# dwofk/fast-depth

Measured on NVIDIA H100. Metric: depth-maps/sec @224x224 b64, higher is better.
Workload: dtype f16

## Files before the change

### fastdepth_b200/_lib.py

```python
import ctypes
import os

HERE = os.path.dirname(os.path.abspath(__file__))
LIB_PATH = os.environ.get('FD_B200_LIB') or os.path.join(HERE, 'libfastdepth_b200.so')

FD_F32, FD_F16, FD_BF16 = 0, 1, 2
FD_STAGE_STEM, FD_STAGE_DWPW, FD_STAGE_HEAD, FD_STAGE_CONV, FD_STAGE_DECONV, FD_STAGE_UPCONV = 0, 1, 2, 3, 4, 5
FD_ACT_RELU, FD_ACT_RELU6 = 0, 1


class StageDesc(ctypes.Structure):
    _fields_ = [(n, ctypes.c_int32) for n in
                ('kind', 'c_in', 'c_out', 'ksize', 'stride', 'act', 'upsample', 'skip_src', 'skip_mode')]


_c_int_p = ctypes.POINTER(ctypes.c_int)
_c_float_p = ctypes.POINTER(ctypes.c_float)
_c_double_p = ctypes.POINTER(ctypes.c_double)
_vp = ctypes.c_void_p

SIGNATURES = {
    'fd_abi_version': (ctypes.c_int, []),
    'fd_last_error': (ctypes.c_char_p, []),
    'fd_plan_create': (ctypes.c_int, [ctypes.POINTER(StageDesc), ctypes.c_int, ctypes.c_int, ctypes.c_int,
                                      ctypes.c_int, ctypes.c_int, ctypes.c_int, ctypes.POINTER(_vp)]),
    'fd_plan_set_stage_weights': (ctypes.c_int, [_vp, ctypes.c_int, _vp, _vp, _vp, _vp, _vp, _vp]),
    'fd_plan_set_option': (ctypes.c_int, [_vp, ctypes.c_char_p, ctypes.c_int]),
    'fd_plan_get_option': (ctypes.c_int, [_vp, ctypes.c_char_p, _c_int_p]),
    'fd_forward': (ctypes.c_int, [_vp, _vp, _vp, _vp]),
    'fd_forward_batch': (ctypes.c_int, [_vp, ctypes.c_int, _vp, _vp, _vp]),
    'fd_forward_shape': (ctypes.c_int, [_vp, ctypes.c_int, ctypes.c_int, ctypes.c_int, _vp, _vp, _vp]),
    'fd_forward_host': (ctypes.c_int, [_vp, _vp, _vp, _vp]),
    'fd_pipeline_submit': (ctypes.c_int, [_vp, _vp, _vp, ctypes.POINTER(ctypes.c_uint64)]),
    'fd_pipeline_wait': (ctypes.c_int, [_vp, ctypes.c_uint64]),
    'fd_stage_buffer': (ctypes.c_int, [_vp, ctypes.c_int, ctypes.c_int, ctypes.POINTER(_vp),
                                       _c_int_p, _c_int_p, _c_int_p, _c_int_p, _c_int_p]),
    'fd_plan_launches_per_forward': (ctypes.c_int, [_vp, _c_int_p]),
    'fd_plan_workspace_bytes': (ctypes.c_int, [_vp, ctypes.POINTER(ctypes.c_size_t)]),
    'fd_plan_step_count': (ctypes.c_int, [_vp, _c_int_p]),
    'fd_plan_step_info': (ctypes.c_int, [_vp, ctypes.c_int, _c_int_p, _c_double_p, _c_double_p,
                                         ctypes.c_char_p, ctypes.c_int]),
    'fd_plan_step_macs': (ctypes.c_int, [_vp, ctypes.c_int, _c_double_p, _c_double_p]),
    'fd_plan_time_steps': (ctypes.c_int, [_vp, _vp, _vp, _vp, ctypes.c_int, ctypes.c_int, ctypes.c_int, _c_float_p]),
    'fd_plan_trace_stage': (ctypes.c_int, [_vp, ctypes.c_int, _vp, _vp, ctypes.POINTER(ctypes.c_uint64), ctypes.c_int,
                                           _c_int_p, _c_int_p]),
    'fd_debug_block_plan': (ctypes.c_int, [ctypes.c_int] * 8 + [_c_int_p, ctypes.c_int]),
    'fd_debug_conv_plan': (ctypes.c_int, [ctypes.c_int] * 7 + [_c_int_p, ctypes.c_int]),
    'fd_debug_convt_plan': (ctypes.c_int, [ctypes.c_int] * 8 + [_c_int_p, ctypes.c_int]),
    'fd_debug_pw_tf32x3_plan': (ctypes.c_int, [ctypes.c_int] * 7 + [_c_int_p, ctypes.c_int]),
    'fd_debug_pw_plan': (ctypes.c_int, [ctypes.c_int] * 7 + [_c_int_p, ctypes.c_int]),
    'fd_debug_conv_tf32x3_plan': (ctypes.c_int, [ctypes.c_int] * 9 + [_c_int_p, ctypes.c_int]),
    'fd_metrics_accumulate': (ctypes.c_int, [_vp, _vp, ctypes.c_int, ctypes.c_int, ctypes.c_int, _vp,
                                             ctypes.c_int, _vp]),
    'fd_nyu_val_gather': (ctypes.c_int, [_vp, _vp, _vp, _vp] + [ctypes.c_int] * 6 + [_vp, _vp, ctypes.c_int, _vp]),
    'fd_plan_destroy': (None, [_vp]),
}

_lib = None


def load():
    global _lib
    if _lib is not None:
        return _lib
    if not os.path.exists(LIB_PATH):
        raise RuntimeError(
            "fastdepth_b200: %s not found. Build it with `python -m fastdepth_b200.build` "
            "(or __graft_entry__.build()); there is no fallback path." % LIB_PATH)
    lib = ctypes.CDLL(LIB_PATH)
    for name, (res, args) in SIGNATURES.items():
# ... 14 lines not shown
```

### fastdepth_b200/build.py

```python
import os
import subprocess
import sys

HERE = os.path.dirname(os.path.abspath(__file__))
CSRC = os.path.join(HERE, 'csrc')
LIB = os.path.join(HERE, 'libfastdepth_b200.so')
SOURCES = ('fd_api.cu', 'fd_kernels_simt.cu', 'fd_block_tc.cu', 'fd_chain_tc.cu', 'fd_stem_tc.cu', 'fd_conv_tc.cu',
           'fd_metrics.cu')
NVCC_FLAGS = ['-gencode', 'arch=compute_90a,code=sm_90a', '-O3', '-lineinfo', '-std=c++17',
              '-Xcompiler', '-fPIC']


def _nvcc():
    for cand in (os.environ.get('NVCC'), '/usr/local/cuda/bin/nvcc', 'nvcc'):
        if cand and (os.path.isabs(cand) and os.path.exists(cand) or not os.path.isabs(cand)):
            return cand
    raise RuntimeError('nvcc not found')


def _stale(target, deps):
    if not os.path.exists(target):
        return True
    t = os.path.getmtime(target)
    return any(os.path.getmtime(d) > t for d in deps)


def build(force=False, verbose=False):
    srcs = [os.path.join(CSRC, s) for s in SOURCES]
    deps = srcs + [os.path.join(CSRC, f) for f in os.listdir(CSRC) if f.endswith(('.cuh', '.h'))]
    deps.append(os.path.join(os.path.dirname(HERE), 'include', 'fastdepth_b200.h'))
# ... 43 lines not shown
```

### fastdepth_b200/csrc/fd_api.cu

```cuda
#include <algorithm>
#include <cstring>
#include <functional>
#include <string>
#include <vector>

#include "fd_block_plan.h"
#include "fd_conv_plan.h"
#include "fd_common.cuh"

namespace fd {

BlockPlanOut block_tc_debug_plan(int ksize, int stride, int h_out, int w_out, int n, int c_in, int c_out, int head);
ConvPlanOut conv_tc_debug_plan(int kind, int ksize, int h_out, int w_out, int n, int c_in, int c_out, int n_sms);
ConvPlanOut pw_tf32x3_debug_plan(int h_out, int w_out, int n, int c_in, int c_out, int upsample, int n_sms);
ConvPlanOut pw_tc_debug_plan(int h_out, int w_out, int n, int c_in, int c_out, int upsample, int n_sms);
ConvPlanOut conv_tc_tf32x3_debug_plan(int kind, int ksize, int h_out, int w_out, int n, int c_in, int c_out, int upsample,
                                      int n_sms);

static thread_local std::string g_last_error;
void set_error(const std::string& msg) { g_last_error = msg; }
int fail(int code, const std::string& msg) {
    g_last_error = msg;
    return code;
}
// ... 13 lines not shown
                          int w_in, int oh, int ow, void* x, float* t, cudaStream_t st);
struct BlockTcPlan;
bool block_tc_supported(int dtype, const StageGeom& g, bool head_fused);
int block_tc_prepare(int dtype, const BlockArgs& a, const float* head_w, float head_scale, float head_bias, int head_act,
                     void* head_out, bool tma_epilogue, const TcLaunchOpts& opts, BlockTcPlan** out);
int block_tc_launch(BlockTcPlan* p, cudaStream_t st, void* head_out);
void block_tc_destroy(BlockTcPlan* p);
const char* block_tc_name(BlockTcPlan* p);
int block_tc_trace(BlockTcPlan* bp, cudaStream_t st, void* head_out, unsigned long long* out_host, int* rows, int* cols);
struct ChainTcPlan;
bool chain_tc_supported(int dtype, const StageGeom* g, int n_layers);
int chain_tc_prepare(int dtype, const BlockArgs* layers, int n_layers, const TcLaunchOpts& opts, ChainTcPlan** out);
int chain_tc_launch(ChainTcPlan* cp, cudaStream_t st);
void chain_tc_destroy(ChainTcPlan* cp);
const char* chain_tc_name(ChainTcPlan* cp);
int chain_tc_trace(ChainTcPlan* cp, cudaStream_t st, unsigned long long* out_host, int* rows, int* cols);
struct StemTcPlan;
bool stem_tc_supported(int dtype, const StageGeom& g);
int stem_tc_prepare(int dtype, const StageGeom& g, const float* w27_dev, const float* scale_dev, const float* bias_dev, void* out,
                    const TcLaunchOpts& opts, StemTcPlan** res);
int stem_tc_launch(StemTcPlan* sp, const void* x, cudaStream_t st);
void stem_tc_destroy(StemTcPlan* sp);
const char* stem_tc_name(StemTcPlan* sp);
struct ConvTcPlan;
bool conv_tc_supported(int dtype, const StageGeom& g, int kind);
int conv_tc_prepare(int dtype, int kind, const StageGeom& g, const void* in, const void* w, const float* scale_dev,
                    const float* bias_dev, void* out, const TcLaunchOpts& opts, ConvTcPlan** res);
int conv_tc_launch(ConvTcPlan* cp, cudaStream_t st);
void conv_tc_destroy(ConvTcPlan* cp);
const char* conv_tc_name(ConvTcPlan* cp);
bool pw_tf32x3_supported(const StageGeom& g);
bool conv_tc_tf32x3_supported(const StageGeom& g, int kind);
int conv_tc_tf32x3_prepare(int kind, const StageGeom& g, const void* in, const float* w_split, const float* scale_dev,
                           const float* bias_dev, void* out, const TcLaunchOpts& opts, ConvTcPlan** res);
int pw_tf32x3_prepare(const StageGeom& g, const void* mid, const float* w_split, const float* scale_dev, const float* bias_dev,
                      void* out, int out_pitch, int reduce, const TcLaunchOpts& opts, ConvTcPlan** res);
int tf32_split_weights(const float* w, size_t count, float* dst);
bool pw_tc_supported(int dtype, const StageGeom& g);
int pw_tc_prepare(int dtype, const StageGeom& g, const void* mid, const void* w, const float* scale_dev, const float* bias_dev,
                  void* out, int out_pitch, int reduce, const TcLaunchOpts& opts, ConvTcPlan** res);
int dw_mid_launch(int dtype, const BlockArgs& a, cudaStream_t st);
BlockPlanOut block_tc_plan_for(const StageGeom& g, const TcLaunchOpts& opts, bool* pinned);
size_t block_tc_param_bytes(BlockTcPlan* bp);
size_t chain_tc_param_bytes(ChainTcPlan* cp);
size_t stem_tc_param_bytes(StemTcPlan* sp);
size_t conv_tc_param_bytes(ConvTcPlan* cp);
// ... 9 lines not shown
    void* out = nullptr;
    void* out_alloc = nullptr;
    int out_c = 0;
    int out_pitch = 0;
    int concat_src = -1;
    void* mid = nullptr;
    float* dw_w = nullptr;
    float* dw_scale = nullptr;
    float* dw_bias = nullptr;
    void* pw_w = nullptr;
    float* pw_w_f32 = nullptr;
    float* pw_scale = nullptr;
    float* pw_bias = nullptr;
    float* w_split = nullptr;
    float head_scale = 0.f, head_bias = 0.f;
    bool have_weights = false;
};

struct StageRun {
    BlockTcPlan* tc = nullptr;
    StemTcPlan* stc = nullptr;
    ConvTcPlan* ctc = nullptr;
    ChainTcPlan* chain = nullptr;
    int chained = 0;
    void* out_eff = nullptr;
};

struct Step {
    int stage;
    std::string name;
    double alg_bytes, macs;
    double dw_macs = 0.0;
    std::function<int(cudaStream_t, const void*, void*)> run;
};

struct StageShape {
    StageGeom g{};
    int out_h = 0, out_w = 0;
    int out_c = 0;
};

struct StepSet {
    int n = 0, h = 0, w = 0;
    std::vector<Step> steps;
    std::vector<StageRun> runs;
    size_t bytes = 0;
    unsigned long long stamp = 0;
};

}

using namespace fd;

struct fd_plan {
    int n = 0, h = 0, w = 0, dtype = 0, device = 0, n_sms = 132;
    std::vector<Stage> stages;
    std::vector<StepSet*> sets;
    unsigned long long set_clock = 0;
    int opt_path = 1, opt_fold_head = 1, opt_graph = 1, opt_tma_epilogue = 1, opt_inplace_skip = 1, opt_pdl = 0, opt_wait_sleep_ns = 0;
    int opt_chain = 1;
    int opt_cluster = 1;
    int opt_tf32x3 = 0;
    int opt_unfuse = 1;
    size_t workspace_bytes = 0;
    size_t split_bytes = 0;
    struct PipeSlot { void* x = nullptr; void* y = nullptr; cudaEvent_t up = nullptr, done = nullptr, down = nullptr; bool busy = false; };
    PipeSlot pipe[3];
    cudaStream_t pipe_h2d = nullptr, pipe_run = nullptr, pipe_d2h = nullptr;
    unsigned long long pipe_next = 0;
    void* stage_x = nullptr;
    void* stage_y = nullptr;
    cudaEvent_t last_done = nullptr;
    cudaStream_t last_stream = nullptr;
    bool last_stream_set = false;
    void* l2_flush = nullptr;
    size_t l2_flush_bytes = 0;
    struct GraphEntry { const void* x; void* y; int n, h, w; cudaGraphExec_t exec; unsigned long long stamp; };
    std::vector<GraphEntry> graphs;
    unsigned long long graph_clock = 0;
    int graph_misses = 0;
};
static const size_t kMaxGraphs = 8;
static const size_t kUnfuseMaxMidBytes = size_t(16) << 20;
static const size_t kMaxStepSets = 8;

namespace fd {
// ... 5 lines not shown
        if (cudaGetDevice(&prev) != cudaSuccess) { ok = false; return; }
        if (prev != dev && cudaSetDevice(dev) != cudaSuccess) ok = false;
    }
    ~DeviceGuard() {
        if (prev >= 0) cudaSetDevice(prev);
    }
};

static int dev_alloc(fd_plan* p, void** ptr, size_t bytes) {
    bytes = (bytes + 255) & ~size_t(255);
    FD_CUDA_OK(cudaMalloc(ptr, bytes));
    FD_CUDA_OK(cudaMemset(*ptr, 0, bytes));
    FD_CUDA_OK(cudaStreamSynchronize(cudaStreamLegacy));
    p->workspace_bytes += bytes;
    return FD_OK;
}

static void destroy_set(StepSet* ss) {
    for (auto& r : ss->runs) {
        if (r.tc) block_tc_destroy(r.tc);
        if (r.stc) stem_tc_destroy(r.stc);
        if (r.ctc) conv_tc_destroy(r.ctc);
        if (r.chain) chain_tc_destroy(r.chain);
    }
    delete ss;
}

static StepSet* find_set(fd_plan* p, int n, int h, int w) {
    for (StepSet* ss : p->sets)
        if (ss->n == n && ss->h == h && ss->w == w) return ss;
    return nullptr;
}

static bool is_capacity_set(const fd_plan* p, const StepSet* ss) { return ss->n == p->n && ss->h == p->h && ss->w == p->w; }

static void invalidate(fd_plan* p) {
    for (auto& g : p->graphs) cudaGraphExecDestroy(g.exec);
    p->graphs.clear();
    for (StepSet* ss : p->sets) destroy_set(ss);
    p->sets.clear();
    for (auto& s : p->stages) { cudaFree(s.w_split); s.w_split = nullptr; }
    p->split_bytes = 0;
}

static int split_weights(fd_plan* p, Stage& s, size_t count, const float** out) {
    if (!s.w_split) {
// ... 67 lines not shown
            s.g.h_out = hh; s.g.w_out = ww;
        }
        s.out_h = s.g.h_out * (s.g.upsample || is_phased(d.kind) ? 2 : 1);
        s.out_w = s.g.w_out * (s.g.upsample || is_phased(d.kind) ? 2 : 1);
        s.out_c = d.c_out;
        if (d.skip_src >= 0) {
            if (d.kind != FD_STAGE_DWPW || !d.upsample || d.skip_src >= i) return fail(FD_ERR_INVALID, "bad skip_src");
            const StageShape& src = out[d.skip_src];
            if (src.out_h != s.out_h || src.out_w != s.out_w || (!d.skip_mode && src.g.c_out != d.c_out))
                return fail(FD_ERR_INVALID, "stage " + std::to_string(i) + ": skip tensor shape does not match the upsampled output");
            if (d.skip_mode) {
                if (d.skip_mode != 1 || concat_src[d.skip_src] >= 0 || stages[d.skip_src].skip_src >= 0)
                    return fail(FD_ERR_INVALID, "bad skip_mode / skip source");
                s.out_c = d.c_out + src.g.c_out;
                concat_src[d.skip_src] = i;
            }
        }
        ch = s.out_c; hh = s.out_h; ww = s.out_w;
    }
    if (hh != h || ww != w) return fail(FD_ERR_INVALID, "stage list does not return to the input resolution");
    return FD_OK;
}

static int build_steps(fd_plan* p, int n, int h, int w, StepSet* ss) {
    const int ns = (int)p->stages.size();
    const double es = (double)dtype_size(p->dtype);
    for (auto& s : p->stages)
        if (!s.have_weights) return fail(FD_ERR_STATE, "fd_plan_set_stage_weights was not called for every stage");
    ss->n = n; ss->h = h; ss->w = w;
    ss->runs.assign(ns, StageRun());
    std::vector<StageRun>& R = ss->runs;
    std::vector<fd_stage_desc> D(ns);
    for (int i = 0; i < ns; ++i) D[i] = p->stages[i].d;
    std::vector<StageShape> S;
    int wrc = walk_stages(D.data(), ns, n, h, w, S);
    if (wrc != FD_OK) return wrc;
    std::vector<StageGeom> G(ns);
    for (int i = 0; i < ns; ++i) G[i] = S[i].g;

    TcLaunchOpts lopts;
    lopts.pdl = p->opt_pdl; lopts.sleep_ns = p->opt_wait_sleep_ns; lopts.n_sms = p->n_sms; lopts.cluster = p->opt_cluster;
    Stage& head = p->stages[ns - 1];
    Stage& last = p->stages[ns - 2];
    const bool fold = p->opt_fold_head && (last.d.kind == FD_STAGE_DWPW || last.d.kind == FD_STAGE_CONV) && last.d.upsample &&
                      last.d.skip_src < 0;
    bool head_fused = false;

    for (int i = 0; i < ns; ++i) {
        Stage& s = p->stages[i];
        StageRun& r = R[i];
        StageGeom& sg = G[i];
        const void* in = i > 0 ? R[i - 1].out_eff : nullptr;
        r.out_eff = s.out;
        sg.in_pitch = i > 0 ? p->stages[i - 1].out_pitch : 0;
        sg.out_pitch = s.out_pitch;
        sg.skip_pitch = (s.d.skip_src >= 0 && !s.d.skip_mode) ? p->stages[s.d.skip_src].out_pitch : s.out_pitch;
        if (s.d.kind == FD_STAGE_STEM) {
            Step st;
            st.stage = i;
            st.name = "stem_kernel";
            st.macs = (double)sg.n * sg.h_out * sg.w_out * sg.c_out * 27.0;
            st.alg_bytes = ((double)sg.n * 3 * sg.h_in * sg.w_in + (double)sg.n * sg.h_out * sg.w_out * sg.c_out) * es +
                           29.0 * sg.c_out * 4;
            Stage* sp = &s;
            const int dtype = p->dtype;
            if (p->opt_path == 1 && stem_tc_supported(dtype, sg)) {
                int rc = stem_tc_prepare(dtype, sg, s.pw_w_f32, s.pw_scale, s.pw_bias, s.out, lopts, &r.stc);
                if (rc != FD_OK) return rc;
                ss->bytes += stem_tc_param_bytes(r.stc);
                st.name = stem_tc_name(r.stc);
                StemTcPlan* stc = r.stc;
                st.run = [stc](cudaStream_t stream, const void* x, void*) { return stem_tc_launch(stc, x, stream); };
            } else {
                const StageGeom g = sg;
                st.run = [sp, dtype, g](cudaStream_t stream, const void* x, void*) {
                    return launch_stem(dtype, x, sp->out, sp->pw_w_f32, sp->pw_scale, sp->pw_bias, g, stream);
                };
            }
            ss->steps.push_back(st);
        } else if (is_conv(s.d.kind)) {
            StageGeom g = sg;
            if (fold && &s == &last) g.upsample = 0;
            const int kind = s.d.kind;
            const double px_in = (double)g.n * g.h_in * g.w_in, px_out = (double)g.n * g.h_out * g.w_out;
            const double kk = (double)g.ksize * g.ksize;
            Step st;
            st.stage = i;
            st.macs = px_out * g.c_in * g.c_out * kk;
            st.dw_macs = 0.0;
// ... 363 lines not shown
        s.head_scale = pw_scale[0];
        s.head_bias = pw_bias[0];
    }
    FD_CUDA_OK(cudaMemcpy(s.pw_scale, pw_scale, (size_t)d.c_out * 4, cudaMemcpyHostToDevice));
    FD_CUDA_OK(cudaMemcpy(s.pw_bias, pw_bias, (size_t)d.c_out * 4, cudaMemcpyHostToDevice));
    s.have_weights = true;
    invalidate(p);
    return FD_OK;
}

static int* option_slot(fd_plan* p, const char* name) {
    if (!p || !name) return nullptr;
    if (!strcmp(name, "path")) return &p->opt_path;
    if (!strcmp(name, "fold_head")) return &p->opt_fold_head;
    if (!strcmp(name, "graph")) return &p->opt_graph;
    if (!strcmp(name, "tma_epilogue")) return &p->opt_tma_epilogue;
    if (!strcmp(name, "inplace_skip")) return &p->opt_inplace_skip;
    if (!strcmp(name, "pdl")) return &p->opt_pdl;
    if (!strcmp(name, "wait_sleep_ns")) return &p->opt_wait_sleep_ns;
    if (!strcmp(name, "chain")) return &p->opt_chain;
    if (!strcmp(name, "cluster")) return &p->opt_cluster;
    if (!strcmp(name, "tf32x3")) return &p->opt_tf32x3;
    if (!strcmp(name, "unfuse")) return &p->opt_unfuse;
    return nullptr;
}

int fd_plan_set_option(fd_plan* p, const char* name, int value) {
    int* slot = option_slot(p, name);
    if (!slot) return fail(FD_ERR_INVALID, std::string("unknown option: ") + (name ? name : "(null)"));
    const bool is_time = !strcmp(name, "wait_sleep_ns");
    if (!strcmp(name, "unfuse")) {
        if (value < 0 || value > 2) return fail(FD_ERR_INVALID, "unfuse must be 0, 1 or 2");
    } else if (is_time ? (value < 0 || value > 100000) : (value != 0 && value != 1)) {
        return fail(FD_ERR_INVALID, is_time ? "wait_sleep_ns must be in [0, 100000]" : "option value must be 0 or 1");
    }
    if (*slot != value) { *slot = value; invalidate(p); }
    return FD_OK;
}

int fd_plan_get_option(fd_plan* p, const char* name, int* value) {
    int* slot = option_slot(p, name);
    if (!slot || !value) return fail(FD_ERR_INVALID, "unknown option or NULL value");
    *value = *slot;
    return FD_OK;
}

// ... 302 lines not shown
int fd_plan_trace_stage(fd_plan* p, int stage, void* y_dev, void* stream, unsigned long long* out_host, int cap, int* rows, int* cols) {
    if (!p || stage < 0 || stage >= (int)p->stages.size() || !out_host || !rows || !cols) return fail(FD_ERR_INVALID, "bad argument");
    DeviceGuard guard(p->device);
    StepSet* ss = nullptr;
    int rc = ensure_steps(p, p->n, p->h, p->w, &ss);
    if (rc) return rc;
    if (cap < 12 * 256) return fail(FD_ERR_INVALID, "trace buffer too small (need 3072 entries)");
    if (is_conv(p->stages[stage].d.kind)) return fail(FD_ERR_INVALID, "the stage timeline exists for fused block kernels only");
    const StageRun& r = ss->runs[stage];
    if (r.chain) return chain_tc_trace(r.chain, (cudaStream_t)stream, out_host, rows, cols);
    if (!r.tc) return fail(FD_ERR_STATE, "stage does not run the fused block kernel");
    return block_tc_trace(r.tc, (cudaStream_t)stream, y_dev, out_host, rows, cols);
}

int fd_debug_block_plan(int ksize, int stride, int h_out, int w_out, int n, int c_in, int c_out, int head, int* out, int cap) {
    if (!out || cap < 16) return fail(FD_ERR_INVALID, "need an int[16] output");
    const BlockPlanOut q = block_tc_debug_plan(ksize, stride, h_out, w_out, n, c_in, c_out, head);
    const int v[16] = {q.ok, q.splits, q.n_cta, q.items, q.kblocks, q.s_in, q.s_a, q.s_b, q.bn, q.nb, q.b_resident, q.n_stg,
                       q.smem_bytes, q.in_stage_stride, q.cs, q.dw_teams};
    for (int i = 0; i < 16; ++i) out[i] = v[i];
    return FD_OK;
}

int fd_debug_conv_plan(int ksize, int h_out, int w_out, int n, int c_in, int c_out, int n_sms, int* out, int cap) {
    if (!out || cap < 16) return fail(FD_ERR_INVALID, "need an int[16] output");
    const ConvPlanOut q = conv_tc_debug_plan(FD_STAGE_CONV, ksize, h_out, w_out, n, c_in, c_out, n_sms);
    const int v[16] = {q.ok, q.ni, q.th, q.tw, q.bn, q.stages, q.m_tiles, q.n_splits, q.items, q.waves, q.kblocks, q.smem_bytes,
                       q.useful_permille, (int)(q.cost > 2e9 ? 2e9 : q.cost), 0, 0};
    for (int i = 0; i < 16; ++i) out[i] = v[i];
    return FD_OK;
}

int fd_debug_pw_plan(int h_out, int w_out, int n, int c_in, int c_out, int upsample, int n_sms, int* out, int cap) {
    if (!out || cap < 16) return fail(FD_ERR_INVALID, "need an int[16] output");
    const ConvPlanOut q = pw_tc_debug_plan(h_out, w_out, n, c_in, c_out, upsample, n_sms);
    const int v[16] = {q.ok, q.ni, q.th, q.tw, q.bn, q.stages, q.m_tiles, q.n_splits, q.items, q.waves, q.kblocks, q.smem_bytes,
                       q.useful_permille, (int)(q.cost > 2e9 ? 2e9 : q.cost), q.ok ? conv_stage_bytes(q.bn) : 0, 0};
    for (int i = 0; i < 16; ++i) out[i] = v[i];
    return FD_OK;
}

int fd_debug_pw_tf32x3_plan(int h_out, int w_out, int n, int c_in, int c_out, int upsample, int n_sms, int* out, int cap) {
    if (!out || cap < 16) return fail(FD_ERR_INVALID, "need an int[16] output");
    const ConvPlanOut q = pw_tf32x3_debug_plan(h_out, w_out, n, c_in, c_out, upsample, n_sms);
    const int v[16] = {q.ok, q.ni, q.th, q.tw, q.bn, q.stages, q.m_tiles, q.n_splits, q.items, q.waves, q.kblocks, q.smem_bytes,
                       q.useful_permille, (int)(q.cost > 2e9 ? 2e9 : q.cost), q.ok ? conv_stage_bytes_tf32x3(q.bn) : 0, 0};
// ... 80 lines not shown
```

### include/fastdepth_b200.h

```cpp
#ifndef FASTDEPTH_B200_H
#define FASTDEPTH_B200_H

#include <stddef.h>
#include <stdint.h>

#ifdef __cplusplus
extern "C" {
#endif

#define FD_ABI_VERSION 2

typedef struct fd_plan fd_plan;

typedef enum {
    FD_OK = 0,
    FD_ERR_INVALID = -1,
    FD_ERR_CUDA = -2,
    FD_ERR_STATE = -3,
    FD_ERR_UNSUPPORTED = -4
} fd_status;

typedef enum { FD_F32 = 0, FD_F16 = 1, FD_BF16 = 2 } fd_dtype;

typedef enum {
// ... 44 lines not shown
                    int* n, int* h, int* w, int* c, int* c_stride);

int fd_plan_launches_per_forward(fd_plan* plan, int* n_launches);
int fd_plan_workspace_bytes(fd_plan* plan, size_t* bytes);
int fd_plan_step_count(fd_plan* plan, int* n_steps);
int fd_plan_step_info(fd_plan* plan, int step, int* stage, double* alg_bytes, double* macs,
                      char* kernel_name, int name_cap);
int fd_plan_step_macs(fd_plan* plan, int step, double* dw_macs, double* dense_macs);
int fd_plan_time_steps(fd_plan* plan, const void* x_dev, void* y_dev, void* stream,
                       int warmup, int iters, int flush_l2, float* ms_out);

int fd_plan_trace_stage(fd_plan* plan, int stage, void* y_dev, void* stream,
                        unsigned long long* out_host, int cap, int* rows, int* cols);

int fd_debug_block_plan(int ksize, int stride, int h_out, int w_out, int n, int c_in, int c_out, int head,
                        int* out, int cap);

int fd_debug_conv_plan(int ksize, int h_out, int w_out, int n, int c_in, int c_out, int n_sms, int* out, int cap);

int fd_debug_pw_tf32x3_plan(int h_out, int w_out, int n, int c_in, int c_out, int upsample, int n_sms, int* out, int cap);

int fd_debug_pw_plan(int h_out, int w_out, int n, int c_in, int c_out, int upsample, int n_sms, int* out, int cap);

int fd_debug_convt_plan(int kind, int ksize, int h_in, int w_in, int n, int c_in, int c_out, int n_sms, int* out, int cap);

int fd_debug_conv_tf32x3_plan(int kind, int ksize, int h, int w, int n, int c_in, int c_out, int upsample, int n_sms,
                              int* out, int cap);

int fd_metrics_accumulate(const void* pred_dev, const float* target_dev, int dtype, int n, int hw,
                          double* sums_dev, int device, void* stream);

int fd_nyu_val_gather(const uint8_t* rgb_dev, const float* depth_dev, const int* rows_dev, const int* cols_dev,
                      int n, int h_in, int w_in, int out_h, int out_w, int dtype,
                      void* x_dev, float* target_dev, int device, void* stream);

void fd_plan_destroy(fd_plan* plan);

const char* fd_last_error(void);
int fd_abi_version(void);

#ifdef __cplusplus
}
#endif
#endif
```

Before: 55680.

## Fuse stem conv and first two depthwise-pointwise blocks into one tensor-core kernel

Adds a front kernel that computes the stride-2 stem conv and the next two dw+pw blocks per 8x8 output tile entirely in shared memory. It uses a TMA input load, WGMMA pointwise GEMMs and halo recomputation, and enables it by default for f16/bf16 FastDepth shapes. The aim is to remove the global-memory round trips and launches between the three earliest, most bandwidth-heavy stages. In exchange it recomputes halo regions, needs a large shared-memory footprint that limits occupancy to two CTAs per SM, and still writes every intermediate output to global memory.

```diff
diff --git a/fastdepth_b200/_lib.py b/fastdepth_b200/_lib.py
--- a/fastdepth_b200/_lib.py
+++ b/fastdepth_b200/_lib.py
@@ -46,6 +46,8 @@
                                            _c_int_p, _c_int_p]),
     'fd_debug_block_plan': (ctypes.c_int, [ctypes.c_int] * 8 + [_c_int_p, ctypes.c_int]),
     'fd_debug_conv_plan': (ctypes.c_int, [ctypes.c_int] * 7 + [_c_int_p, ctypes.c_int]),
+    'fd_debug_front_plan': (ctypes.c_int, [_vp, ctypes.c_int, ctypes.c_int, ctypes.c_int, ctypes.c_int, ctypes.c_int,
+                                           _c_int_p, ctypes.c_int]),
     'fd_debug_convt_plan': (ctypes.c_int, [ctypes.c_int] * 8 + [_c_int_p, ctypes.c_int]),
     'fd_debug_pw_tf32x3_plan': (ctypes.c_int, [ctypes.c_int] * 7 + [_c_int_p, ctypes.c_int]),
     'fd_debug_pw_plan': (ctypes.c_int, [ctypes.c_int] * 7 + [_c_int_p, ctypes.c_int]),
diff --git a/fastdepth_b200/build.py b/fastdepth_b200/build.py
--- a/fastdepth_b200/build.py
+++ b/fastdepth_b200/build.py
@@ -5,7 +5,7 @@
 HERE = os.path.dirname(os.path.abspath(__file__))
 CSRC = os.path.join(HERE, 'csrc')
 LIB = os.path.join(HERE, 'libfastdepth_b200.so')
-SOURCES = ('fd_api.cu', 'fd_kernels_simt.cu', 'fd_block_tc.cu', 'fd_chain_tc.cu', 'fd_stem_tc.cu', 'fd_conv_tc.cu',
+SOURCES = ('fd_api.cu', 'fd_kernels_simt.cu', 'fd_block_tc.cu', 'fd_chain_tc.cu', 'fd_stem_tc.cu', 'fd_front_tc.cu', 'fd_conv_tc.cu',
            'fd_metrics.cu')
 NVCC_FLAGS = ['-gencode', 'arch=compute_90a,code=sm_90a', '-O3', '-lineinfo', '-std=c++17',
               '-Xcompiler', '-fPIC']
diff --git a/fastdepth_b200/csrc/fd_api.cu b/fastdepth_b200/csrc/fd_api.cu
--- a/fastdepth_b200/csrc/fd_api.cu
+++ b/fastdepth_b200/csrc/fd_api.cu
@@ -59,6 +59,17 @@
 int stem_tc_launch(StemTcPlan* sp, const void* x, cudaStream_t st);
 void stem_tc_destroy(StemTcPlan* sp);
 const char* stem_tc_name(StemTcPlan* sp);
+struct FrontTcPlan;
+bool front_tc_shape_ok(int dtype, const StageGeom& g0, const StageGeom& g1, const StageGeom& g2);
+int front_tc_items(int n, int h, int w);
+void front_tc_layout(int* out);
+int front_tc_prepare(int dtype, const StageGeom& g0, const StageGeom& g1, const StageGeom& g2, const float* w27,
+                     const float* sc0, const float* bi0, const BlockArgs& a1, const BlockArgs& a2, void* out0,
+                     const TcLaunchOpts& opts, FrontTcPlan** res);
+int front_tc_launch(FrontTcPlan* fp, const void* x, cudaStream_t st);
+void front_tc_destroy(FrontTcPlan* fp);
+const char* front_tc_name(FrontTcPlan* fp);
+size_t front_tc_param_bytes(FrontTcPlan* fp);
 struct ConvTcPlan;
 bool conv_tc_supported(int dtype, const StageGeom& g, int kind);
 int conv_tc_prepare(int dtype, int kind, const StageGeom& g, const void* in, const void* w, const float* scale_dev,
@@ -114,6 +125,7 @@
     StemTcPlan* stc = nullptr;
     ConvTcPlan* ctc = nullptr;
     ChainTcPlan* chain = nullptr;
+    FrontTcPlan* front = nullptr;
     int chained = 0;
     void* out_eff = nullptr;
 };
@@ -154,6 +166,7 @@
     int opt_cluster = 1;
     int opt_tf32x3 = 0;
     int opt_unfuse = 1;
+    int opt_front = 1;
     size_t workspace_bytes = 0;
     size_t split_bytes = 0;
     struct PipeSlot { void* x = nullptr; void* y = nullptr; cudaEvent_t up = nullptr, done = nullptr, down = nullptr; bool busy = false; };
@@ -205,6 +218,7 @@
         if (r.stc) stem_tc_destroy(r.stc);
         if (r.ctc) conv_tc_destroy(r.ctc);
         if (r.chain) chain_tc_destroy(r.chain);
+        if (r.front) front_tc_destroy(r.front);
     }
     delete ss;
 }
@@ -318,6 +332,14 @@
     return FD_OK;
 }
 
+static bool front_route_ok(const fd_stage_desc* D, int ns, int dtype, const std::vector<StageShape>& S) {
+    if (ns < 4 || D[0].kind != FD_STAGE_STEM || D[1].kind != FD_STAGE_DWPW || D[2].kind != FD_STAGE_DWPW) return false;
+    if (D[1].skip_src >= 0 || D[2].skip_src >= 0) return false;
+    for (int j = 3; j < ns; ++j)
+        if (D[j].skip_src >= 0 && D[j].skip_src <= 2 && D[j].skip_mode) return false;
+    return front_tc_shape_ok(dtype, S[0].g, S[1].g, S[2].g);
+}
+
 static int build_steps(fd_plan* p, int n, int h, int w, StepSet* ss) {
     const int ns = (int)p->stages.size();
     const double es = (double)dtype_size(p->dtype);
@@ -360,7 +382,37 @@
                            29.0 * sg.c_out * 4;
             Stage* sp = &s;
             const int dtype = p->dtype;
-            if (p->opt_path == 1 && stem_tc_supported(dtype, sg)) {
+            if (p->opt_path == 1 && p->opt_front && front_route_ok(D.data(), ns, dtype, S) && stem_tc_supported(dtype, sg)) {
+                BlockArgs a[2]{};
+                StageGeom g[3] = {sg, G[1], G[2]};
+                for (int k = 1; k <= 2; ++k) {
+                    Stage& t = p->stages[k];
+                    g[k].in_pitch = p->stages[k - 1].out_pitch; g[k].out_pitch = t.out_pitch;
+                    BlockArgs& b = a[k - 1];
+                    b.g = g[k]; b.out = t.out;
+                    b.dw_w = t.dw_w; b.dw_scale = t.dw_scale; b.dw_bias = t.dw_bias;
+                    b.pw_w = t.pw_w; b.pw_scale = t.pw_scale; b.pw_bias = t.pw_bias;
+                }
+                int rc = front_tc_prepare(dtype, g[0], g[1], g[2], s.pw_w_f32, s.pw_scale, s.pw_bias, a[0], a[1], s.out, lopts, &r.front);
+                if (rc != FD_OK) return rc;
+                ss->bytes += front_tc_param_bytes(r.front);
+                st.stage = 2;
+                st.name = front_tc_name(r.front);
+                st.dw_macs = 0.0;
+                double wb = 29.0 * sg.c_out * 4, out_px_bytes = (double)sg.n * sg.h_out * sg.w_out * sg.c_out;
+                for (int k = 1; k <= 2; ++k) {
+                    const double px = (double)g[k].n * g[k].h_out * g[k].w_out;
+                    st.dw_macs += px * g[k].c_in * 9.0;
+                    st.macs += px * g[k].c_in * 9.0 + px * g[k].c_in * g[k].c_out;
+                    wb += (double)g[k].c_in * 9 * 4 + 2.0 * g[k].c_in * 4 + (double)g[k].c_in * g[k].c_out * es + 2.0 * g[k].c_out * 4;
+                    out_px_bytes += px * g[k].c_out;
+                    R[k].chained = 1;
+                    R[k].out_eff = p->stages[k].out;
+                }
+                st.alg_bytes = ((double)sg.n * 3 * sg.h_in * sg.w_in + out_px_bytes) * es + wb;
+                FrontTcPlan* fp = r.front;
+                st.run = [fp](cudaStream_t stream, const void* x, void*) { return front_tc_launch(fp, x, stream); };
+            } else if (p->opt_path == 1 && stem_tc_supported(dtype, sg)) {
                 int rc = stem_tc_prepare(dtype, sg, s.pw_w_f32, s.pw_scale, s.pw_bias, s.out, lopts, &r.stc);
                 if (rc != FD_OK) return rc;
                 ss->bytes += stem_tc_param_bytes(r.stc);
@@ -770,6 +822,7 @@
     if (!strcmp(name, "cluster")) return &p->opt_cluster;
     if (!strcmp(name, "tf32x3")) return &p->opt_tf32x3;
     if (!strcmp(name, "unfuse")) return &p->opt_unfuse;
+    if (!strcmp(name, "front")) return &p->opt_front;
     return nullptr;
 }
 
@@ -1118,6 +1171,19 @@
     return FD_OK;
 }
 
+int fd_debug_front_plan(const fd_stage_desc* stages, int n_stages, int dtype, int n, int h, int w, int* out, int cap) {
+    if (!out || cap < 8) return fail(FD_ERR_INVALID, "need an int[8] output");
+    if (!stages || n_stages < 1) return fail(FD_ERR_INVALID, "no stages");
+    std::vector<StageShape> S;
+    const int rc = walk_stages(stages, n_stages, n, h, w, S);
+    if (rc != FD_OK) return rc;
+    const bool ok = front_route_ok(stages, n_stages, dtype, S);
+    out[0] = ok ? 1 : 0;
+    out[1] = ok ? front_tc_items(n, h, w) : 0;
+    front_tc_layout(out + 2);
+    return FD_OK;
+}
+
 int fd_debug_conv_plan(int ksize, int h_out, int w_out, int n, int c_in, int c_out, int n_sms, int* out, int cap) {
     if (!out || cap < 16) return fail(FD_ERR_INVALID, "need an int[16] output");
     const ConvPlanOut q = conv_tc_debug_plan(FD_STAGE_CONV, ksize, h_out, w_out, n, c_in, c_out, n_sms);
diff --git a/fastdepth_b200/csrc/fd_front_tc.cu b/fastdepth_b200/csrc/fd_front_tc.cu
--- /dev/null
+++ b/fastdepth_b200/csrc/fd_front_tc.cu
@@ -0,0 +1,456 @@
+#include <cstdio>
+#include <cstring>
+#include <new>
+#include <string>
+
+#include "fd_tc_common.cuh"
+
+namespace fd {
+
+constexpr int FR_THREADS = 256;
+constexpr int FR_C0 = 32, FR_C1 = 64, FR_C2 = 128;
+constexpr int FR_T0 = 19, FR_T1 = 17, FR_T2 = 8;
+constexpr int FR_XH = 39, FR_XW = 48;
+constexpr int FR_X_BYTES = 3 * FR_XH * FR_XW * 2;
+constexpr int FR_A0_ROWS = 192;
+constexpr uint32_t FR_W0 = 0, FR_W1 = FR_W0 + FR_C0 * 128, FR_W2 = FR_W1 + FR_C1 * 128;
+constexpr uint32_t FR_R1 = FR_W2 + FR_C2 * 128;
+constexpr uint32_t FR_X = FR_R1 + 28672;
+constexpr uint32_t FR_R2 = FR_R1 + 320 * 128;
+constexpr uint32_t FR_PRM = FR_R2 + 37120;
+constexpr uint32_t FR_P_TAP1 = 0, FR_P_SB1 = FR_P_TAP1 + 9 * FR_C0 * 2, FR_P_TAP2 = FR_P_SB1 + 2 * FR_C0 * 4;
+constexpr uint32_t FR_P_SB2 = FR_P_TAP2 + 9 * FR_C1 * 2, FR_P_AFF0 = FR_P_SB2 + 2 * FR_C1 * 4;
+constexpr uint32_t FR_P_AFF1 = FR_P_AFF0 + FR_C0 * 8, FR_P_AFF2 = FR_P_AFF1 + FR_C1 * 8, FR_P_BYTES = FR_P_AFF2 + FR_C2 * 8;
+constexpr uint32_t FR_BAR = FR_PRM + FR_P_BYTES;
+constexpr uint32_t FR_W_BYTES = (FR_C0 + FR_C1 + FR_C2) * 128;
+
+struct FrontParams {
+    int n, h, w;
+    int tiles_x, tiles_y, items;
+    int pitch0, pitch1, pitch2;
+    void* out0;
+    void* out1;
+    void* out2;
+    const uint4* blob;
+};
+
+size_t front_tc_smem_bytes() { return (size_t)FR_BAR + 8 + 1024; }
+void front_tc_layout(int* out) {
+    out[0] = (int)front_tc_smem_bytes(); out[1] = 2; out[2] = FR_THREADS;
+    out[3] = (int)(FR_R1 - FR_W0 + FR_P_BYTES); out[4] = (int)(FR_R2 - FR_R1); out[5] = (int)(FR_PRM - FR_R2);
+    static_assert(FR_X + FR_X_BYTES <= FR_R2 && FR_X >= FR_R1 + FR_A0_ROWS * 128, "x box beside the stem chunk, inside the A region");
+}
+
+template <typename T, bool RELU6>
+__global__ void __launch_bounds__(FR_THREADS, 2)
+front_tc_kernel(const __grid_constant__ CUtensorMap tm_x, const FrontParams p) {
+    using MF = MixFma<T>;
+    extern __shared__ uint8_t smem_raw[];
+    const uint32_t smem_base = (smem_u32(smem_raw) + 1023u) & ~1023u;
+    uint8_t* smem = smem_raw + (smem_base - smem_u32(smem_raw));
+    uint8_t* r1 = smem + FR_R1;
+    uint8_t* r2 = smem + FR_R2;
+    const uint8_t* prm = smem + FR_PRM;
+    const uint32_t bar = smem_base + FR_BAR;
+    const int tid = threadIdx.x, warp = tid >> 5, lane = tid & 31;
+    const int wg = warp >> 2, wq = warp & 3, cq = (lane & 3) * 2;
+    const int h0 = p.h >> 1, w0 = p.w >> 1, h2 = p.h >> 2, w2 = p.w >> 2;
+
+    if (tid == 0) { mbar_init(bar, 1); fence_barrier_init(); tma_prefetch_desc(&tm_x); }
+    for (int i = tid; i < (int)(FR_W_BYTES / 16); i += FR_THREADS) {
+        const int r = i >> 3, c = i & 7;
+        *reinterpret_cast<uint4*>(smem + r * 128 + ((c ^ (r & 7)) << 4)) = p.blob[i];
+    }
+    for (int i = tid; i < (int)(FR_P_BYTES / 16); i += FR_THREADS)
+        reinterpret_cast<uint4*>(smem + FR_PRM)[i] = p.blob[FR_W_BYTES / 16 + i];
+    fence_proxy_async();
+    pdl_launch_dependents();
+    pdl_wait_prior_grid();
+    __syncthreads();
+
+    auto decode = [&](int it, int& img, int& oy2, int& ox2) {
+        const int t = it / p.tiles_x;
+        ox2 = (it - t * p.tiles_x) * FR_T2;
+        img = t / p.tiles_y;
+        oy2 = (t - img * p.tiles_y) * FR_T2;
+    };
+    auto load_x = [&](int it) {
+        int img, oy2, ox2;
+        decode(it, img, oy2, ox2);
+        mbar_expect_tx(bar, FR_X_BYTES);
+        tma_load_4d(smem_base + FR_X, &tm_x, bar, 4 * ox2 - 8, 4 * oy2 - 5, 0, img);
+    };
+    if (tid == 0 && (int)blockIdx.x < p.items) load_x(blockIdx.x);
+
+    const int q1 = lane & 15;
+    const float* sb1 = reinterpret_cast<const float*>(prm + FR_P_SB1);
+    const float* sb2 = reinterpret_cast<const float*>(prm + FR_P_SB2);
+    const float2* aff0 = reinterpret_cast<const float2*>(prm + FR_P_AFF0);
+    const float2* aff1 = reinterpret_cast<const float2*>(prm + FR_P_AFF1);
+    const float2* aff2 = reinterpret_cast<const float2*>(prm + FR_P_AFF2);
+    const uint32_t w_lo = sw128_desc_lo(smem_base);
+    const uint32_t r1_lo = sw128_desc_lo(smem_base + FR_R1);
+    T* __restrict__ o0 = reinterpret_cast<T*>(p.out0);
+    T* __restrict__ o1 = reinterpret_cast<T*>(p.out1);
+    T* __restrict__ o2 = reinterpret_cast<T*>(p.out2);
+
+    uint32_t ph = 0;
+    for (int it = blockIdx.x; it < p.items; it += gridDim.x, ph ^= 1u) {
+        int img, oy2, ox2;
+        decode(it, img, oy2, ox2);
+        const int y0 = 2 * oy2 - 2, x0 = 2 * ox2 - 2;
+        const int y1 = 2 * oy2 - 1, x1 = 2 * ox2 - 1;
+        mbar_wait(bar, ph);
+
+        for (int ch = 0; ch < 2; ++ch) {
+            if (tid < FR_A0_ROWS) {
+                const int m = ch * FR_A0_ROWS + tid;
+                uint32_t wd[16];
+                if (m < FR_T0 * FR_T0) {
+                    const int ty = m / FR_T0, tx = m - ty * FR_T0;
+                    const uint8_t* xs = smem + FR_X + (2 * ty * FR_XW + 2 * tx + 2) * 2;
+                    uint32_t hv[27];
+#pragma unroll
+                    for (int r = 0; r < 9; ++r) {
+                        const int ci = r / 3, ky = r % 3;
+                        const uint32_t* q = reinterpret_cast<const uint32_t*>(xs + ((ci * FR_XH + ky) * FR_XW) * 2);
+                        const uint32_t v0 = q[0], v1 = q[1];
+                        hv[3 * r] = v0 >> 16; hv[3 * r + 1] = v1 & 0xffffu; hv[3 * r + 2] = v1 >> 16;
+                    }
+#pragma unroll
+                    for (int j = 0; j < 16; ++j) {
+                        const uint32_t lo = (2 * j < 27) ? hv[(2 * j < 27) ? 2 * j : 0] : 0u;
+                        const uint32_t hi = (2 * j + 1 < 27) ? hv[(2 * j + 1 < 27) ? 2 * j + 1 : 0] : 0u;
+                        wd[j] = lo | (hi << 16);
+                    }
+                } else {
+#pragma unroll
+                    for (int j = 0; j < 16; ++j) wd[j] = 0u;
+                }
+                uint8_t* a_row = r1 + tid * 128;
+#pragma unroll
+                for (int c = 0; c < 4; ++c)
+                    *reinterpret_cast<uint4*>(a_row + ((c ^ (tid & 7)) << 4)) = make_uint4(wd[4 * c], wd[4 * c + 1], wd[4 * c + 2], wd[4 * c + 3]);
+            }
+            fence_proxy_async();
+            __syncthreads();
+            for (int mb = wg; mb < 3; mb += 2) {
+                float acc[16];
+                wgmma_fence();
+                wgmma_n32<T>(acc, sw128_desc(r1_lo + (uint32_t)mb * 512u), sw128_desc(w_lo + (FR_W0 >> 4)), 0u);
+                wgmma_n32<T>(acc, sw128_desc(r1_lo + (uint32_t)mb * 512u + 2u), sw128_desc(w_lo + (FR_W0 >> 4) + 2u), 1u);
+                wgmma_commit();
+                wgmma_wait0();
+#pragma unroll
+                for (int h = 0; h < 2; ++h) {
+                    const int m = ch * FR_A0_ROWS + mb * 64 + wq * 16 + (lane >> 2) + 8 * h;
+                    if (m >= FR_T0 * FR_T0) continue;
+                    const int ty = m / FR_T0, tx = m - ty * FR_T0;
+                    const bool in_map = (unsigned)(y0 + ty) < (unsigned)h0 && (unsigned)(x0 + tx) < (unsigned)w0;
+                    uint8_t* row = r2 + m * 64;
+#pragma unroll
+                    for (int i = 0; i < 4; ++i) {
+                        const float4 af = *reinterpret_cast<const float4*>(aff0 + i * 8 + cq);
+                        const uint32_t v = in_map ? MF::template pack_act<true>(ffma2_abc(f32x2_make(acc[4 * i + 2 * h], acc[4 * i + 2 * h + 1]),
+                                                                                          f32x2_make(af.x, af.y), f32x2_make(af.z, af.w)))
+                                                  : 0u;
+                        *reinterpret_cast<uint32_t*>(row + ((i ^ ((m >> 1) & 3)) << 4) + cq * 2) = v;
+                    }
+                }
+            }
+            __syncthreads();
+        }
+
+        for (int i = tid; i < 16 * 16 * 4; i += FR_THREADS) {
+            const int px = i >> 2, c = i & 3, ty = 2 + (px >> 4), tx = 2 + (px & 15), m = ty * FR_T0 + tx;
+            const uint4 v = *reinterpret_cast<const uint4*>(r2 + m * 64 + ((c ^ ((m >> 1) & 3)) << 4));
+            *reinterpret_cast<uint4*>(o0 + (((size_t)img * h0 + y0 + ty) * w0 + x0 + tx) * p.pitch0 + c * 8) = v;
+        }
+        f32x2 k1[9];
+#pragma unroll
+        for (int t = 0; t < 9; ++t) k1[t] = MF::widen(*reinterpret_cast<const uint32_t*>(prm + FR_P_TAP1 + (t * FR_C0 + 2 * q1) * 2));
+        const f32x2 s1 = f32x2_make(sb1[2 * q1], sb1[2 * q1 + 1]), b1 = f32x2_make(sb1[FR_C0 + 2 * q1], sb1[FR_C0 + 2 * q1 + 1]);
+        {
+            const int uy = tid >> 4;
+            f32x2 acc[FR_T1];
+#pragma unroll
+            for (int o = 0; o < FR_T1; ++o) acc[o] = 0ull;
+#pragma unroll
+            for (int ky = 0; ky < 3; ++ky) {
+                const int mrow = (uy + ky) * FR_T0;
+#pragma unroll
+                for (int ix = 0; ix < FR_T0; ++ix) {
+                    const int mi = mrow + ix;
+                    const f32x2 v = MF::widen(*reinterpret_cast<const uint32_t*>(r2 + mi * 64 + (((q1 >> 2) ^ ((mi >> 1) & 3)) << 4) + (q1 & 3) * 4));
+#pragma unroll
+                    for (int kx = 0; kx < 3; ++kx)
+                        if (ix - kx >= 0 && ix - kx < FR_T1) ffma2(acc[ix - kx], v, k1[ky * 3 + kx]);
+                }
+            }
+#pragma unroll
+            for (int o = 0; o < FR_T1; ++o) {
+                const int m = uy * FR_T1 + o;
+                uint8_t* a_row = r1 + m * 128;
+                *reinterpret_cast<uint32_t*>(a_row + (((q1 >> 2) ^ (m & 7)) << 4) + (q1 & 3) * 4) = MF::template pack_act<RELU6>(ffma2_abc(acc[o], s1, b1));
+                *reinterpret_cast<uint32_t*>(a_row + ((((q1 >> 2) + 4) ^ (m & 7)) << 4) + (q1 & 3) * 4) = 0u;
+            }
+        }
+        for (int u = tid; u < FR_T1 * 16; u += FR_THREADS) {
+            const int ux = u >> 4, m = (FR_T1 - 1) * FR_T1 + ux;
+            f32x2 acc = 0ull;
+#pragma unroll
+            for (int ky = 0; ky < 3; ++ky)
+#pragma unroll
+                for (int kx = 0; kx < 3; ++kx) {
+                    const int mi = (FR_T1 - 1 + ky) * FR_T0 + ux + kx;
+                    ffma2(acc, MF::widen(*reinterpret_cast<const uint32_t*>(r2 + mi * 64 + (((q1 >> 2) ^ ((mi >> 1) & 3)) << 4) + (q1 & 3) * 4)),
+                          k1[ky * 3 + kx]);
+                }
+            uint8_t* a_row = r1 + m * 128;
+            *reinterpret_cast<uint32_t*>(a_row + (((q1 >> 2) ^ (m & 7)) << 4) + (q1 & 3) * 4) = MF::template pack_act<RELU6>(ffma2_abc(acc, s1, b1));
+            *reinterpret_cast<uint32_t*>(a_row + ((((q1 >> 2) + 4) ^ (m & 7)) << 4) + (q1 & 3) * 4) = 0u;
+        }
+        fence_proxy_async();
+        __syncthreads();
+
+        for (int mb = wg; mb < 5; mb += 2) {
+            float acc[32];
+            wgmma_fence();
+#pragma unroll
+            for (int k4 = 0; k4 < 4; ++k4)
+                wgmma_n64<T>(acc, sw128_desc(r1_lo + (uint32_t)mb * 512u + 2u * k4), sw128_desc(w_lo + (FR_W1 >> 4) + 2u * k4), k4 > 0 ? 1u : 0u);
+            wgmma_commit();
+            wgmma_wait0();
+#pragma unroll
+            for (int h = 0; h < 2; ++h) {
+                const int m = mb * 64 + wq * 16 + (lane >> 2) + 8 * h;
+                if (m >= FR_T1 * FR_T1) continue;
+                const int uy = m / FR_T1, ux = m - uy * FR_T1;
+                const bool in_map = (unsigned)(y1 + uy) < (unsigned)h0 && (unsigned)(x1 + ux) < (unsigned)w0;
+                uint8_t* row = r2 + m * 128;
+#pragma unroll
+                for (int i = 0; i < 8; ++i) {
+                    const float4 af = *reinterpret_cast<const float4*>(aff1 + i * 8 + cq);
+                    const uint32_t v = in_map ? MF::template pack_act<RELU6>(ffma2_abc(f32x2_make(acc[4 * i + 2 * h], acc[4 * i + 2 * h + 1]),
+                                                                                      f32x2_make(af.x, af.y), f32x2_make(af.z, af.w)))
+                                              : 0u;
+                    *reinterpret_cast<uint32_t*>(row + ((i ^ (m & 7)) << 4) + cq * 2) = v;
+                }
+            }
+        }
+        __syncthreads();
+        if (tid == 0 && it + (int)gridDim.x < p.items) load_x(it + gridDim.x);
+
+        for (int i = tid; i < 16 * 16 * 8; i += FR_THREADS) {
+            const int px = i >> 3, c = i & 7, uy = 1 + (px >> 4), ux = 1 + (px & 15), m = uy * FR_T1 + ux;
+            const uint4 v = *reinterpret_cast<const uint4*>(r2 + m * 128 + ((c ^ (m & 7)) << 4));
+            *reinterpret_cast<uint4*>(o1 + (((size_t)img * h0 + y1 + uy) * w0 + x1 + ux) * p.pitch1 + c * 8) = v;
+        }
+        {
+            const int vy = tid >> 5;
+            f32x2 k2[9];
+#pragma unroll
+            for (int t = 0; t < 9; ++t) k2[t] = MF::widen(*reinterpret_cast<const uint32_t*>(prm + FR_P_TAP2 + (t * FR_C1 + 2 * lane) * 2));
+            const f32x2 s2 = f32x2_make(sb2[2 * lane], sb2[2 * lane + 1]), b2 = f32x2_make(sb2[FR_C1 + 2 * lane], sb2[FR_C1 + 2 * lane + 1]);
+            f32x2 acc[FR_T2];
+#pragma unroll
+            for (int o = 0; o < FR_T2; ++o) acc[o] = 0ull;
+#pragma unroll
+            for (int ky = 0; ky < 3; ++ky) {
+                const int mrow = (2 * vy + ky) * FR_T1;
+#pragma unroll
+                for (int ix = 0; ix < FR_T1; ++ix) {
+                    const int mi = mrow + ix;
+                    const f32x2 v = MF::widen(*reinterpret_cast<const uint32_t*>(r2 + mi * 128 + (((lane >> 2) ^ (mi & 7)) << 4) + (lane & 3) * 4));
+#pragma unroll
+                    for (int kx = 0; kx < 3; ++kx)
+                        if (((ix - kx) & 1) == 0 && ix - kx >= 0 && (ix - kx) / 2 < FR_T2) ffma2(acc[(ix - kx) / 2], v, k2[ky * 3 + kx]);
+                }
+            }
+#pragma unroll
+            for (int o = 0; o < FR_T2; ++o) {
+                const int m = vy * FR_T2 + o;
+                *reinterpret_cast<uint32_t*>(r1 + m * 128 + (((lane >> 2) ^ (m & 7)) << 4) + (lane & 3) * 4) =
+                    MF::template pack_act<RELU6>(ffma2_abc(acc[o], s2, b2));
+            }
+        }
+        fence_proxy_async();
+        __syncthreads();
+
+        {
+            float acc[32];
+            wgmma_fence();
+#pragma unroll
+            for (int k4 = 0; k4 < 4; ++k4)
+                wgmma_n64<T>(acc, sw128_desc(r1_lo + 2u * k4), sw128_desc(w_lo + (FR_W2 >> 4) + (uint32_t)wg * 512u + 2u * k4), k4 > 0 ? 1u : 0u);
+            wgmma_commit();
+            wgmma_wait0();
+#pragma unroll
+            for (int h = 0; h < 2; ++h) {
+                const int m = wq * 16 + (lane >> 2) + 8 * h;
+                uint8_t* row = r2 + m * 256;
+#pragma unroll
+                for (int i = 0; i < 8; ++i) {
+                    const int c = wg * 8 + i;
+                    const float4 af = *reinterpret_cast<const float4*>(aff2 + c * 8 + cq);
+                    *reinterpret_cast<uint32_t*>(row + ((c ^ (m & 15)) << 4) + cq * 2) = MF::template pack_act<RELU6>(
+                        ffma2_abc(f32x2_make(acc[4 * i + 2 * h], acc[4 * i + 2 * h + 1]), f32x2_make(af.x, af.y), f32x2_make(af.z, af.w)));
+                }
+            }
+        }
+        __syncthreads();
+        for (int i = tid; i < 64 * 16; i += FR_THREADS) {
+            const int m = i >> 4, c = i & 15;
+            const uint4 v = *reinterpret_cast<const uint4*>(r2 + m * 256 + ((c ^ (m & 15)) << 4));
+            *reinterpret_cast<uint4*>(o2 + (((size_t)img * h2 + oy2 + (m >> 3)) * w2 + ox2 + (m & 7)) * p.pitch2 + c * 8) = v;
+        }
+    }
+}
+
+struct FrontTcPlan {
+    CUtensorMap tm_x;
+    FrontParams p;
+    dim3 grid;
+    size_t smem_bytes;
+    int dtype, relu6;
+    TcLaunchOpts opts;
+    const void* x_bound = nullptr;
+    void* blob = nullptr;
+    std::string name;
+};
+
+bool front_tc_shape_ok(int dtype, const StageGeom& g0, const StageGeom& g1, const StageGeom& g2) {
+    if (dtype != FD_F16 && dtype != FD_BF16) return false;
+    if (g0.ksize != 3 || g0.stride != 2 || g0.c_in != 3 || g0.c_out != FR_C0 || g0.act != FD_ACT_RELU6 || g0.upsample) return false;
+    if (g0.h_in % 32 || g0.w_in % 32) return false;
+    if (g1.ksize != 3 || g1.stride != 1 || g1.c_in != FR_C0 || g1.c_out != FR_C1 || g1.upsample) return false;
+    if (g2.ksize != 3 || g2.stride != 2 || g2.c_in != FR_C1 || g2.c_out != FR_C2 || g2.upsample) return false;
+    return g1.act == g2.act;
+}
+
+int front_tc_items(int n, int h, int w) { return n * (h / 32) * (w / 32); }
+
+template <typename T>
+__global__ void pack_front_kernel(const float* __restrict__ w27, const T* __restrict__ pw1, const T* __restrict__ pw2,
+                                  const float* __restrict__ sc0, const float* __restrict__ bi0,
+                                  const float* __restrict__ dw1, const float* __restrict__ dsc1, const float* __restrict__ dbi1,
+                                  const float* __restrict__ sc1, const float* __restrict__ bi1,
+                                  const float* __restrict__ dw2, const float* __restrict__ dsc2, const float* __restrict__ dbi2,
+                                  const float* __restrict__ sc2, const float* __restrict__ bi2, uint8_t* __restrict__ blob) {
+    const int i = blockIdx.x * blockDim.x + threadIdx.x;
+    T* wt = reinterpret_cast<T*>(blob);
+    if (i < (FR_C0 + FR_C1 + FR_C2) * 64) {
+        const int r = i / 64, k = i % 64;
+        if (r < FR_C0) wt[i] = Traits<T>::from_f(k < 27 ? w27[k * FR_C0 + r] : 0.f);
+        else if (r < FR_C0 + FR_C1) wt[i] = k < FR_C0 ? pw1[(r - FR_C0) * FR_C0 + k] : Traits<T>::from_f(0.f);
+        else wt[i] = pw2[(r - FR_C0 - FR_C1) * FR_C1 + k];
+    }
+    uint8_t* prm = blob + FR_W_BYTES;
+    if (i < 9 * FR_C0) reinterpret_cast<T*>(prm + FR_P_TAP1)[i] = Traits<T>::from_f(dw1[i]);
+    if (i < 9 * FR_C1) reinterpret_cast<T*>(prm + FR_P_TAP2)[i] = Traits<T>::from_f(dw2[i]);
+    if (i < FR_C0) { reinterpret_cast<float*>(prm + FR_P_SB1)[i] = dsc1[i]; reinterpret_cast<float*>(prm + FR_P_SB1)[FR_C0 + i] = dbi1[i]; }
+    if (i < FR_C1) { reinterpret_cast<float*>(prm + FR_P_SB2)[i] = dsc2[i]; reinterpret_cast<float*>(prm + FR_P_SB2)[FR_C1 + i] = dbi2[i]; }
+    auto aff = [&](uint32_t off, const float* s, const float* b, int c) {
+        float* d = reinterpret_cast<float*>(prm + off) + (c >> 1) * 4;
+        d[c & 1] = s[c];
+        d[2 + (c & 1)] = b[c];
+    };
+    if (i < FR_C0) aff(FR_P_AFF0, sc0, bi0, i);
+    if (i < FR_C1) aff(FR_P_AFF1, sc1, bi1, i);
+    if (i < FR_C2) aff(FR_P_AFF2, sc2, bi2, i);
+}
+
+void front_tc_destroy(FrontTcPlan* fp) {
+    if (!fp) return;
+    cudaFree(fp->blob);
+    delete fp;
+}
+
+static int encode_front_x(FrontTcPlan* fp, const void* x) {
+    PFN_encodeTiled encode = get_tensor_map_encoder();
+    const CUtensorMapDataType dt = fp->dtype == FD_F16 ? CU_TENSOR_MAP_DATA_TYPE_FLOAT16 : CU_TENSOR_MAP_DATA_TYPE_BFLOAT16;
+    const FrontParams& p = fp->p;
+    cuuint64_t dims[4] = {(cuuint64_t)p.w, (cuuint64_t)p.h, 3, (cuuint64_t)p.n};
+    cuuint64_t strides[3] = {(cuuint64_t)p.w * 2, (cuuint64_t)p.w * p.h * 2, (cuuint64_t)p.w * p.h * 6};
+    cuuint32_t box[4] = {FR_XW, FR_XH, 3, 1};
+    cuuint32_t estr[4] = {1, 1, 1, 1};
+    CUresult r = encode(&fp->tm_x, dt, 4, const_cast<void*>(x), dims, strides, box, estr, CU_TENSOR_MAP_INTERLEAVE_NONE,
+                        CU_TENSOR_MAP_SWIZZLE_NONE, CU_TENSOR_MAP_L2_PROMOTION_L2_128B, CU_TENSOR_MAP_FLOAT_OOB_FILL_NONE);
+    if (r != CUDA_SUCCESS) return fail(FD_ERR_CUDA, "cuTensorMapEncodeTiled(front input) failed: " + std::to_string((int)r));
+    fp->x_bound = x;
+    return FD_OK;
+}
+
+int front_tc_prepare(int dtype, const StageGeom& g0, const StageGeom& g1, const StageGeom& g2, const float* w27,
+                     const float* sc0, const float* bi0, const BlockArgs& a1, const BlockArgs& a2, void* out0,
+                     const TcLaunchOpts& opts, FrontTcPlan** res) {
+    FrontTcPlan* fp = new (std::nothrow) FrontTcPlan();
+    if (!fp) return fail(FD_ERR_CUDA, "out of host memory");
+    fp->dtype = dtype; fp->relu6 = g1.act == FD_ACT_RELU6; fp->opts = opts;
+    FrontParams& p = fp->p;
+    memset(&p, 0, sizeof(p));
+    p.n = g0.n; p.h = g0.h_in; p.w = g0.w_in;
+    p.tiles_x = g2.w_out / FR_T2; p.tiles_y = g2.h_out / FR_T2; p.items = p.tiles_x * p.tiles_y * p.n;
+    p.pitch0 = g0.out_pitch; p.pitch1 = g1.out_pitch; p.pitch2 = g2.out_pitch;
+    p.out0 = out0; p.out1 = a1.out; p.out2 = a2.out;
+    const size_t blob_bytes = FR_W_BYTES + FR_P_BYTES;
+    if (cudaMalloc(&fp->blob, blob_bytes) != cudaSuccess) { front_tc_destroy(fp); return fail(FD_ERR_CUDA, "cudaMalloc failed"); }
+    const int tot = (FR_C0 + FR_C1 + FR_C2) * 64;
+    if (dtype == FD_F16)
+        pack_front_kernel<__half><<<(tot + 127) / 128, 128>>>(w27, (const __half*)a1.pw_w, (const __half*)a2.pw_w, sc0, bi0, a1.dw_w, a1.dw_scale,
+                                                              a1.dw_bias, a1.pw_scale, a1.pw_bias, a2.dw_w, a2.dw_scale, a2.dw_bias,
+                                                              a2.pw_scale, a2.pw_bias, (uint8_t*)fp->blob);
+    else
+        pack_front_kernel<__nv_bfloat16><<<(tot + 127) / 128, 128>>>(w27, (const __nv_bfloat16*)a1.pw_w, (const __nv_bfloat16*)a2.pw_w, sc0, bi0,
+                                                                     a1.dw_w, a1.dw_scale, a1.dw_bias, a1.pw_scale, a1.pw_bias, a2.dw_w,
+                                                                     a2.dw_scale, a2.dw_bias, a2.pw_scale, a2.pw_bias, (uint8_t*)fp->blob);
+    if (cudaGetLastError() != cudaSuccess || cudaDeviceSynchronize() != cudaSuccess) {
+        front_tc_destroy(fp);
+        return fail(FD_ERR_CUDA, "front parameter packing failed");
+    }
+    p.blob = reinterpret_cast<const uint4*>(fp->blob);
+    fp->smem_bytes = front_tc_smem_bytes();
+    const int ctas = 2 * opts.n_sms;
+    fp->grid = dim3((unsigned)(p.items < ctas ? p.items : ctas), 1, 1);
+    fp->name = std::string("stem_tc+front<k3s1,k3s2,8x8>[n32,n64,n128,") + (fp->relu6 ? "relu6]" : "relu]");
+    *res = fp;
+    return FD_OK;
+}
+
+size_t front_tc_param_bytes(FrontTcPlan*) { return FR_W_BYTES + FR_P_BYTES; }
+const char* front_tc_name(FrontTcPlan* fp) { return fp->name.c_str(); }
+
+template <typename T, bool R6>
+static int launch_front(FrontTcPlan* fp, cudaLaunchConfig_t& cfg) {
+    static PerDeviceOnce attr_done;
+    int dev = -1;
+    FD_CUDA_OK(cudaGetDevice(&dev));
+    if (attr_done.need(dev)) {
+        FD_CUDA_OK(cudaFuncSetAttribute(front_tc_kernel<T, R6>, cudaFuncAttributeMaxDynamicSharedMemorySize, (int)fp->smem_bytes));
+        attr_done.done(dev);
+    }
+    FD_CUDA_OK(cudaLaunchKernelEx(&cfg, front_tc_kernel<T, R6>, fp->tm_x, fp->p));
+    return FD_OK;
+}
+
+int front_tc_launch(FrontTcPlan* fp, const void* x, cudaStream_t st) {
+    if ((reinterpret_cast<uintptr_t>(x) & 15) != 0) return fail(FD_ERR_INVALID, "stem input must be 16-byte aligned");
+    if (x != fp->x_bound) {
+        int rc = encode_front_x(fp, x);
+        if (rc) return rc;
+    }
+    cudaLaunchConfig_t cfg{};
+    cfg.gridDim = fp->grid; cfg.blockDim = dim3(FR_THREADS); cfg.dynamicSmemBytes = fp->smem_bytes; cfg.stream = st;
+    cudaLaunchAttribute attr[1];
+    attr[0].id = cudaLaunchAttributeProgrammaticStreamSerialization;
+    attr[0].val.programmaticStreamSerializationAllowed = 1;
+    cfg.attrs = attr; cfg.numAttrs = fp->opts.pdl ? 1 : 0;
+    int rc;
+    if (fp->dtype == FD_F16) rc = fp->relu6 ? launch_front<__half, true>(fp, cfg) : launch_front<__half, false>(fp, cfg);
+    else rc = fp->relu6 ? launch_front<__nv_bfloat16, true>(fp, cfg) : launch_front<__nv_bfloat16, false>(fp, cfg);
+    if (rc) return rc;
+    FD_CUDA_OK(cudaGetLastError());
+    return FD_OK;
+}
+
+}
diff --git a/include/fastdepth_b200.h b/include/fastdepth_b200.h
--- a/include/fastdepth_b200.h
+++ b/include/fastdepth_b200.h
@@ -90,6 +90,8 @@
 
 int fd_debug_pw_plan(int h_out, int w_out, int n, int c_in, int c_out, int upsample, int n_sms, int* out, int cap);
 
+int fd_debug_front_plan(const fd_stage_desc* stages, int n_stages, int dtype, int n, int h, int w, int* out, int cap);
+
 int fd_debug_convt_plan(int kind, int ksize, int h_in, int w_in, int n, int c_in, int c_out, int n_sms, int* out, int cap);
 
 int fd_debug_conv_tf32x3_plan(int kind, int ksize, int h, int w, int n, int c_in, int c_out, int upsample, int n_sms,
```

Result: faster. 58150 (median of 6 runs) (+4.4%).
